# jamieapps101/Basic_Sparse_Matrix

Hardware: AMD Instinct MI355X
Metric: CSR x dense SpMM effective GB/s (B_alg / step time); nnz/s (higher is better)
Workload: dtype f64

## Files before the change

basic_sparse_matrix_amd/_lib.py:

```python

from __future__ import annotations

import ctypes
import os
import threading

import numpy as np

try:
    import torch
except Exception:
    torch = None

LIB_PATH = os.environ.get("BSM_LIB_PATH") or os.path.join(os.path.dirname(os.path.abspath(__file__)), "lib",
                                                          "libbsm_hip.so")

BSM_F64, BSM_F32, BSM_I32, BSM_U32, BSM_I64, BSM_U64 = range(6)
DTYPE_CODES = {
    np.dtype(np.float64): BSM_F64,
    np.dtype(np.float32): BSM_F32,
    np.dtype(np.int32): BSM_I32,
    np.dtype(np.uint32): BSM_U32,
    np.dtype(np.int64): BSM_I64,
    np.dtype(np.uint64): BSM_U64,
# ... 81 lines not shown
    ("bsm_dev_gen_row_ptr", _int, [_u64, _u64, _u64, _u32, _int, _u32, _u32, _vp, _vp, _u64, _vp]),
    ("bsm_dev_gen_entries", _int, [_int, _u64, _u64, _u64, _u32, _int, _vp, _vp, _vp, _vp]),
    ("bsm_dev_gen_dense", _int, [_int, _u64, _u64, _u64, _u64, _int, _vp, _vp]),
    ("bsm_dev_gen_insert_stream", _int, [_int, _u64, _u64, _u64, _u64, _u64, _u64, _vp, _vp, _vp, _vp]),
    ("bsm_dev_csr_from_inserts", _int, [_int, _u64, _u64, _u64, _vp, _vp, _vp, ctypes.POINTER(_vp), _vp]),
    ("bsm_dev_scan_workspace_bytes", _u64, [_u64]),
    ("bsm_dev_spmm", _int, [_int, _u64, _u64, _u64, _vp, _vp, _vp, _u64, _vp, _vp, _vp, _vp]),
    ("bsm_csr_panel_cols", _int, [_vp, _u64p]),
    ("bsm_dev_spmm_panel_cols", _u64, [_int, _u64, _u64]),
    ("bsm_dev_spmm_plan_bytes", _u64, [_u64, _u64, _u64]),
    ("bsm_dev_spmm_plan", _int, [_u64, _u64, _vp, _vp, _u64, _vp, ctypes.POINTER(_int), _vp]),
    ("bsm_dev_spmm_panelled", _int, [_int, _u64, _u64, _u64, _vp, _vp, _vp, _u64, _vp, _vp, _vp, _u64, _vp, _vp]),
    ("bsm_dev_tiled_wanted", _int, [_int, _u64, _u64, _u64, _u64, _u64]),
    ("bsm_dev_tiled_create", _int, [_u64, _u64, _u64, _vp, _vp, _vp, _u64, _int, ctypes.POINTER(_vp), _vp]),
    ("bsm_dev_spmm_tiled", _int, [_vp, _vp, _vp, _vp, _vp]),
    ("bsm_tiled_info", _int, [_vp, _u64p, _u64p, _u64p]),
    ("bsm_tiled_destroy", None, [_vp]),
    ("bsm_csr_tiled", _int, [_vp, ctypes.POINTER(_int)]),
    ("bsm_xfer_counters", _int, [_u64p]),
    ("bsm_xfer_counters_reset", None, []),
    ("bsm_dev_compact", _int, [_int, _u64, _u64, _vp, _vp, _vp, _vp, _vp, _vp, _u64, _vp]),
    ("bsm_multi_create", _int, [_int, ctypes.POINTER(_int), ctypes.POINTER(_vp)]),
    ("bsm_multi_unique_id", _int, [_vp]),
    ("bsm_multi_create_rank", _int, [_vp, _int, _int, _int, ctypes.POINTER(_vp)]),
    ("bsm_multi_create_external", _int, [_int, _int, _int, ctypes.POINTER(_vp)]),
    ("bsm_multi_is_external", _int, [_vp, ctypes.POINTER(_int)]),
    ("bsm_partition_rows", _int, [_vp, _u64, _u32, _vp]),
    ("bsm_multi_info", _int, [_vp, ctypes.POINTER(_int), ctypes.POINTER(_int), ctypes.POINTER(_int)]),
    ("bsm_multi_broadcast", _int, [_vp, _pp, _u64, _int]),
    ("bsm_multi_destroy", None, [_vp]),
    ("bsm_mcsr_upload", _int, [_vp, _int, _u64, _u64, _u64, _vp, _vp, _vp, _u32, ctypes.POINTER(_vp)]),
# ... 180 lines not shown
```

basic_sparse_matrix_amd/csrc/bsm_internal.hpp:

```cpp
#pragma once

#include <hip/hip_runtime.h>

#include <chrono>
#include <cstdint>
#include <cstdio>
#include <cstring>
#include <memory>
#include <mutex>
#include <string>

#include "../../include/bsm.h"

namespace bsm {

void set_error(const char* fmt, ...);
const char* last_error();
void stage_reset(hipStream_t s);
void stage_mark(const char* name, hipStream_t s);

#define BSM_HIP_TRY(expr)                                                                   \
    do {                                                                                    \
        hipError_t bsm_e_ = (expr);                                                         \
        if (bsm_e_ != hipSuccess) {                                                         \
// ... 132 lines not shown
        bytes = 0;
        cap = 0;
        return q;
    }
    template <typename T> T* as() const { return static_cast<T*>(p); }
};

}

struct bsm_tiled {
    int device = 0;
    int dtype = BSM_F64;
    uint64_t k = 32;
    uint32_t overread = 4;
    uint32_t stage = 4;
    uint64_t rows = 0, n_cols = 0, nnz = 0;
    uint32_t nw = 0, rpw = 0, nb = 0, rw = 0, pshift = 0;
    uint64_t chunks = 0;
    int64_t* offs = nullptr;
    void* meta = nullptr;
    uint32_t meta_bytes = 4;
    void* val = nullptr;
    unsigned* bar = nullptr;
};

struct bsm_csr {
    int dtype = BSM_F64;
    int device = 0;
    uint64_t rows = 0, cols = 0, nnz = 0;
    int64_t* row_ptr = nullptr;
// ... 68 lines not shown
                            const uint64_t* col, const void* vals, bsm_csr** out, hipStream_t s);
int sparse_addsub_dispatch(const bsm_csr* a, const bsm_csr* b, bool sub, bsm_csr** out, hipStream_t s);
int sparse_mul_dispatch(const bsm_csr* a, const bsm_csr* b, bsm_csr** out, hipStream_t s);
int csr_from_coo_device(int dtype, uint64_t rows, uint64_t cols, uint64_t n, const uint64_t* row,
                        const uint64_t* col, const void* vals, bsm_csr** out, hipStream_t s);
int gen_insert_stream(int dtype, uint64_t seed, uint64_t i0, uint64_t n, uint64_t rows, uint64_t cols,
                      uint64_t vmod, uint64_t* row, uint64_t* col, void* vals, hipStream_t s);
uint64_t spmm_panel_cols(int dtype, uint64_t n_cols, uint64_t k);
uint64_t spmm_plan_bytes(uint64_t rows, uint64_t n_cols, uint64_t panel_cols);
int spmm_plan(uint64_t rows, uint64_t n_cols, const int64_t* rp, const int32_t* col,
              uint64_t panel_cols, int32_t* seg, int* usable, hipStream_t s);
int spmm_panelled(int dtype, uint64_t rows, uint64_t n_cols, uint64_t nnz, const int64_t* rp,
                  const int32_t* col, const void* vals, uint64_t k, const void* x, void* y,
                  int32_t* row_nnz, uint64_t panel_cols, const int32_t* seg, hipStream_t s);
bool tiled_wanted(int dtype, uint64_t rows, uint64_t n_cols, uint64_t nnz, uint64_t k, uint64_t max_row_len);
int tiled_create(int dtype, uint64_t rows, uint64_t n_cols, uint64_t nnz, const int64_t* rp, const int32_t* col,
                 const void* vals, uint64_t k, int flags, bsm_tiled** out, hipStream_t s, uint64_t reserve = 0,
                 PlanTimes* pt = nullptr);
int tiled_spmm(const bsm_tiled* t, const void* x, void* y, int32_t* row_nnz, bool neg_init, hipStream_t s);
void tiled_destroy(bsm_tiled* t);
int compact_dispatch(int dtype, uint64_t rows, uint64_t k, const void* y, const int64_t* out_rp,
                     int32_t* out_col, void* out_vals, hipStream_t s);
constexpr uint64_t SMALL_OUT_ROWS = 8192;
constexpr uint64_t SMALL_OUT_CAP = 131072;
inline size_t small_col_bytes(uint64_t cap) { return (cap * sizeof(int32_t) + 15) / 16 * 16; }
int compact_small_dispatch(int dtype, uint64_t rows, uint64_t k, const int32_t* nz, const void* y, int64_t* out_rp,
                           int32_t* out_col, void* out_vals, void* host, uint64_t cap, hipStream_t s);
int pack_cols_to_rowmajor(int dtype, uint64_t n, uint64_t k, const void* colmajor, void* rowmajor,
                          hipStream_t s);
int unpack_rowmajor_to_cols(int dtype, uint64_t n, uint64_t k, const void* rowmajor,
// ... 29 lines not shown
```

basic_sparse_matrix_amd/csrc/capi.hip:

```cpp
#include <atomic>
#include <cstdarg>
#include <cstdlib>
#include <mutex>
#include <vector>

#include <algorithm>
#include <cstring>

#include "bsm_internal.hpp"

namespace bsm {

static thread_local std::string g_err;

void set_error(const char* fmt, ...) {
    char buf[1024];
    va_list ap;
    va_start(ap, fmt);
    vsnprintf(buf, sizeof(buf), fmt, ap);
    va_end(ap);
    g_err = buf;
}
const char* last_error() { return g_err.c_str(); }

// ... 1172 lines not shown
int bsm_dev_tiled_wanted(int dtype, uint64_t rows, uint64_t n_cols, uint64_t nnz, uint64_t k,
                         uint64_t max_row_len) {
    return tiled_wanted(dtype, rows, n_cols, nnz, k, max_row_len) ? 1 : 0;
}

int bsm_dev_tiled_create(uint64_t rows, uint64_t n_cols, uint64_t nnz, const int64_t* row_ptr,
                         const int32_t* col, const double* vals, uint64_t k, int flags, bsm_tiled** out,
                         void* stream) {
    return tiled_create(BSM_F64, rows, n_cols, nnz, row_ptr, col, vals, k, flags, out, static_cast<hipStream_t>(stream));
}

int bsm_dev_spmm_tiled(const bsm_tiled* t, const double* x, double* y, int32_t* row_nnz, void* stream) {
    return tiled_spmm(t, x, y, row_nnz, false, static_cast<hipStream_t>(stream));
}

int bsm_tiled_info(const bsm_tiled* t, uint64_t* bytes, uint64_t* slots, uint64_t* panel_cols) {
    BSM_REQUIRE(t, BSM_ERR_INVALID, "null argument");
    const uint64_t n = (t->chunks + t->overread) * 64;
    if (bytes) *bytes = n * (t->meta_bytes + (t->dtype == BSM_F32 ? 4 : 8)) + ((uint64_t)t->nw * t->nb + 1) * 8;
    if (slots) *slots = t->chunks * 64;
    if (panel_cols) *panel_cols = 1ull << t->pshift;
    return BSM_OK;
}

void bsm_tiled_destroy(bsm_tiled* t) { tiled_destroy(t); }

int bsm_csr_tiled(const bsm_csr* m, int* in_use) {
    BSM_REQUIRE(m && in_use, BSM_ERR_INVALID, "null argument");
    std::lock_guard<std::mutex> lock(m->plan_mu);
    *in_use = m->tiled ? 1 : 0;
    return BSM_OK;
}
// ... 12 lines not shown
```

basic_sparse_matrix_amd/csrc/kernels_tiled.hip:

```cpp
#include "bsm_internal.hpp"

#include <cstdlib>
#include <type_traits>
#include <utility>
#include <vector>


namespace bsm {
namespace {

constexpr int WAVE = 64;
constexpr int CHUNK = 64;
constexpr int PHASES = 6;
constexpr int OVERREAD = 4;
constexpr uint32_t DONE = 0xffffffffu;
constexpr uint32_t RW_MAX = 155;
constexpr uint32_t RW_MAX_F32 = 255;
constexpr uint32_t PSHIFT = 12;
constexpr uint32_t PACE_PCT = 3;

__device__ __forceinline__ uint64_t lanemask_lt(int lane) {
    return lane == 0 ? 0ull : (~0ull >> (64 - lane));
}
__device__ __forceinline__ uint32_t wave_min_u32(uint32_t v) {
#pragma unroll
    for (int off = 1; off < WAVE; off <<= 1) v = min(v, (uint32_t)__shfl_xor((int)v, off, WAVE));
    return v;
}

template <bool WRITE, int SLOTS, typename V, typename M = uint32_t>
__global__ __launch_bounds__(256) void tiled_layout(uint64_t rows, uint64_t n_cols, double pace, uint32_t rbits,
                                                    uint32_t pad, const int64_t* __restrict__ rp,
                                                    const int32_t* __restrict__ col,
                                                    const V* __restrict__ vals, uint32_t nw,
                                                    uint32_t rpw, uint32_t nb, uint32_t rw, uint32_t pshift,
                                                    int32_t* __restrict__ counts,
                                                    const int64_t* __restrict__ offs,
                                                    M* __restrict__ meta, V* __restrict__ val) {
    const int lane = threadIdx.x & (WAVE - 1);
    const uint64_t task = (uint64_t)blockIdx.x * (blockDim.x / WAVE) + threadIdx.x / WAVE;
    if (task >= (uint64_t)nw * nb) return;
    const uint64_t gw = task / nb, b = task % nb;
    const uint64_t w0 = gw * rpw;
    const uint64_t wend = min<uint64_t>(rows, w0 + rpw);
    const uint64_t r0 = w0 + b * rw;
// ... 1 lines not shown
    uint32_t h[SLOTS];
#pragma unroll
    for (int j = 0; j < SLOTS; ++j) {
        const uint32_t s = lane + WAVE * j;
        const bool live = s < rw && r0 + s < wend;
        cur[j] = live ? rp[r0 + s] : 0;
        end[j] = live ? rp[r0 + s + 1] : 0;
        h[j] = cur[j] < end[j] ? (uint32_t)col[cur[j]] >> pshift : DONE;
    }
    const bool any = r0 < wend;
    const int64_t t0 = any ? rp[r0] : 0, t1 = any ? rp[min<uint64_t>(r0 + rw, wend)] : 0;
    const double np = (double)(((n_cols - 1) >> pshift) + 1);
    const double inv_r = t1 > t0 ? (double)CHUNK * np / ((double)(t1 - t0) * pace) : 1e30;
    int64_t c = WRITE ? offs[task] : 0;
    int64_t n = 0;
    for (;;) {
        bool sel[SLOTS];
        int pos[SLOTS];
#pragma unroll
        for (int j = 0; j < SLOTS; ++j) {
            sel[j] = false;
            pos[j] = 0;
        }
        int taken = 0;
        const double pm = (double)n * inv_r;
        const uint32_t pmax = pm >= 4.0e9 ? DONE - 1 : (uint32_t)pm;
        bool done = false;
        while (taken < CHUNK) {
            uint32_t m = DONE;
#pragma unroll
            for (int j = 0; j < SLOTS; ++j) m = min(m, sel[j] ? DONE : h[j]);
            m = wave_min_u32(m);
            if (m == DONE) {
                done = taken == 0;
                break;
            }
            if (m > pmax) break;
            int before = 0;
#pragma unroll
            for (int j = 0; j < SLOTS; ++j) {
                const bool cand = !sel[j] && h[j] == m;
                const uint64_t bal = __ballot(cand);
                const int rank = before + __popcll(bal & lanemask_lt(lane));
                if (cand && taken + rank < CHUNK) {
                    sel[j] = true;
                    pos[j] = taken + rank;
                }
                before += __popcll(bal);
            }
            taken = min(taken + before, CHUNK);
        }
        if (done) break;
#pragma unroll
        for (int j = 0; j < SLOTS; ++j) {
            if (sel[j]) {
                const int64_t e = cur[j];
                if (WRITE) {
                    meta[c * CHUNK + pos[j]] = ((M)(uint32_t)col[e] << rbits) | (M)(lane + WAVE * j);
                    val[c * CHUNK + pos[j]] = vals[e];
                }
                cur[j] = e + 1;
                h[j] = cur[j] < end[j] ? (uint32_t)col[cur[j]] >> pshift : DONE;
            }
        }
        if (WRITE && lane >= taken) {
            meta[c * CHUNK + lane] = (M)rw;
            val[c * CHUNK + lane] = (V)0;
        }
        ++c;
        ++n;
    }
    const int64_t padded = (n + pad - 1) / pad * pad;
    if (WRITE) {
        for (int64_t p = n; p < padded; ++p, ++c) {
            meta[c * CHUNK + lane] = (M)rw;
            val[c * CHUNK + lane] = (V)0;
        }
    } else if (lane == 0) {
        counts[task] = (int32_t)padded;
    }
}

template <typename T> struct Vec2;
template <> struct Vec2<double> { using type = double2; };
struct F2 {
    uint64_t u;
};
template <> struct Vec2<float> { using type = F2; };
__device__ __forceinline__ double lo_of(const double2& v) { return v.x; }
__device__ __forceinline__ double hi_of(const double2& v) { return v.y; }
// ... 140 lines not shown
}

template <bool PROBE, typename T = double, typename M = uint32_t>
__global__ __launch_bounds__(256) __attribute__((amdgpu_waves_per_eu(1, 1))) void spmm_tiled_k32(
    uint64_t rows, uint32_t rpw, uint32_t nb, uint32_t rw, const int64_t* __restrict__ offs,
    const M* __restrict__ meta, const T* __restrict__ val, const vec2_t<T>* __restrict__ X,
    vec2_t<T>* __restrict__ Y, int32_t* __restrict__ row_nnz, unsigned* bar, uint32_t xmask, uint32_t spins) {
    spmm_tiled_k32_body<PROBE, T, M>(rows, rpw, nb, rw, offs, meta, val, X, Y, row_nnz, bar, xmask, spins);
}
template <typename M = uint32_t>
__global__ __launch_bounds__(256) __attribute__((amdgpu_waves_per_eu(1, 1))) void spmm_tiled_k32_f32(
    uint64_t rows, uint32_t rpw, uint32_t nb, uint32_t rw, const int64_t* __restrict__ offs,
    const M* __restrict__ meta, const float* __restrict__ val, const F2* __restrict__ X, F2* __restrict__ Y,
    int32_t* __restrict__ row_nnz, unsigned* bar, uint32_t xmask, uint32_t spins) {
    spmm_tiled_k32_body<false, float, M>(rows, rpw, nb, rw, offs, meta, val, X, Y, row_nnz, bar, xmask, spins);
}

constexpr int K1_STAGE_DEFAULT = 4;
constexpr uint32_t K1_RBITS = 11;
constexpr uint32_t K1_RW_MAX = (1u << K1_RBITS) - 1;
constexpr uint32_t K1_PSHIFT = 18;
constexpr uint32_t K1_WAVES_PER_CU = 4;

template <int ST, typename T>
struct Stage1 {
    uint32_t m[ST];
    T v[ST];
    T x[ST];
};
template <int ST, typename T>
// ... 96 lines not shown

bool tiled_wanted(int dtype, uint64_t rows, uint64_t n_cols, uint64_t nnz, uint64_t k, uint64_t max_row_len) {
    const bool shape = (dtype == BSM_F64 || dtype == BSM_F32) && rows > 0 && nnz > 0 &&
                       ((k == 32 && n_cols <= 0x7fffffffull) || (k == 1 && n_cols < (1u << (32 - K1_RBITS))));
    if (const char* e = getenv("BSM_SPMM_TILED")) {
        if (atoi(e) == 0) return false;
        if (atoi(e) == 2) return shape;
    }
    if (!shape) return false;
    const uint64_t x_bytes = n_cols * k * (dtype == BSM_F32 ? 4 : 8);
    if (x_bytes <= (k == 32 ? (1ull << 30) : (4ull << 20))) return false;
    const uint64_t mean = (nnz + rows - 1) / rows;
    return max_row_len <= 2 * mean + 256;
}

int tiled_create(int dtype, uint64_t rows, uint64_t n_cols, uint64_t nnz, const int64_t* rp, const int32_t* col,
                 const void* vals, uint64_t k, int flags, bsm_tiled** out, hipStream_t s, uint64_t reserve,
                 PlanTimes* pt) {
    BSM_REQUIRE(out && rp && (nnz == 0 || (col && vals)), BSM_ERR_INVALID, "tiled: null argument");
    BSM_REQUIRE(k == 32 || k == 1, BSM_ERR_UNSUPPORTED, "tiled: k must be 32 or 1");
    BSM_REQUIRE(dtype == BSM_F64 || dtype == BSM_F32, BSM_ERR_UNSUPPORTED, "tiled: f64 or f32 only");
    const bool f32 = dtype == BSM_F32;
    const size_t es = f32 ? 4 : 8;
    const bool wide = k == 32 && n_cols >= (1ull << 24);
    const size_t mb = wide ? 8 : 4;
    const uint32_t rbits = k == 1 ? K1_RBITS : 8;
    BSM_REQUIRE(k == 32 ? n_cols <= 0x7fffffffull : n_cols < (1ull << (32 - rbits)), BSM_ERR_UNSUPPORTED,
                "tiled: columns must be < 2^%u", k == 32 ? 31u : 32 - rbits);
    *out = nullptr;
    int dev = 0;
// ... 2 lines not shown
    BSM_HIP_TRY(hipDeviceGetAttribute(&cus, hipDeviceAttributeMultiprocessorCount, dev));
    if (s && cus > 0) {
        std::vector<uint32_t> mk((size_t)(cus + 31) / 32, 0u);
        if (hipExtStreamGetCUMask(s, (uint32_t)mk.size(), mk.data()) == hipSuccess) {
            int n = 0;
            for (int i = 0; i < cus; ++i) n += (mk[i / 32] >> (i % 32)) & 1u;
            if (n > 0 && n < cus) cus = n;
        } else {
            (void)hipGetLastError();
        }
    }
    const uint32_t wpc = k == 1 ? K1_WAVES_PER_CU : 4u;
    const uint32_t nw_env = env_u32("BSM_TILED_WAVES", wpc * (uint32_t)cus);
    const uint32_t nw = nw_env;
    const uint32_t k1_stage = env_u32("BSM_TILED_K1_STAGE", K1_STAGE_DEFAULT) == 8 ? 8u : 4u;
    const uint32_t rw_cap =
        k == 1 ? K1_RW_MAX : (f32 ? RW_MAX_F32 : RW_MAX);
    uint32_t rw_max = env_u32("BSM_TILED_RW", rw_cap);
    rw_max = rw_max < 8u ? 8u : (rw_max > rw_cap ? rw_cap : rw_max);
    const uint32_t pshift = env_u32("BSM_TILED_PSHIFT", k == 1 ? K1_PSHIFT : PSHIFT);
    const double pace = 1.0 + env_u32("BSM_TILED_PACE_PCT", PACE_PCT) / 100.0;
    const uint32_t pad = k == 1 ? 1u : PHASES;
    const uint32_t overread = k == 1 ? 2 * k1_stage : OVERREAD;
    BSM_REQUIRE(nw >= wpc && nw % wpc == 0 && pshift < 32, BSM_ERR_INVALID, "tiled: bad geometry");
    const uint64_t rpw64 = (rows + nw - 1) / nw;
    BSM_REQUIRE(rpw64 < (1ull << 31), BSM_ERR_UNSUPPORTED, "tiled: too many rows per wave");
    const uint32_t rpw = rpw64 ? (uint32_t)rpw64 : 1u;
    const uint32_t nb = (rpw + rw_max - 1) / rw_max;
    const uint32_t rw = (rpw + nb - 1) / nb;
    const uint64_t tasks = (uint64_t)nw * nb;

    DBuf counts, offs, ws;
    BSM_TRY(counts.alloc(tasks * sizeof(int32_t)));
    BSM_TRY(offs.alloc((tasks + 1) * sizeof(int64_t)));
    const uint64_t grid = (tasks + 3) / 4;
    auto layout = [&](auto write_tag, int32_t* cnt, const int64_t* of, void* me, void* va) -> int {
        constexpr bool W = decltype(write_tag)::value;
        auto go = [&]<typename V, typename MT>(V*, MT*) {
            if (k == 1)
                tiled_layout<W, (K1_RW_MAX + 1) / WAVE, V, MT><<<dim3((unsigned)grid), 256, 0, s>>>(
                    rows, n_cols, pace, rbits, pad, rp, col, static_cast<const V*>(vals), nw, rpw, nb, rw, pshift,
                    cnt, of, static_cast<MT*>(me), static_cast<V*>(va));
            else if (rw_cap > 192)
                tiled_layout<W, 4, V, MT><<<dim3((unsigned)grid), 256, 0, s>>>(
                    rows, n_cols, pace, rbits, pad, rp, col, static_cast<const V*>(vals), nw, rpw, nb, rw, pshift,
                    cnt, of, static_cast<MT*>(me), static_cast<V*>(va));
            else
                tiled_layout<W, 3, V, MT><<<dim3((unsigned)grid), 256, 0, s>>>(
                    rows, n_cols, pace, rbits, pad, rp, col, static_cast<const V*>(vals), nw, rpw, nb, rw, pshift,
                    cnt, of, static_cast<MT*>(me), static_cast<V*>(va));
        };
        if (f32 && wide) go((float*)nullptr, (uint64_t*)nullptr);
        else if (f32) go((float*)nullptr, (uint32_t*)nullptr);
        else if (wide) go((double*)nullptr, (uint64_t*)nullptr);
        else go((double*)nullptr, (uint32_t*)nullptr);
        BSM_HIP_TRY(hipGetLastError());
        return BSM_OK;
    };
// ... 36 lines not shown
    auto* t = new bsm_tiled;
    t->device = dev;
    t->dtype = dtype;
    t->k = k;
    t->rows = rows;
    t->n_cols = n_cols;
    t->nnz = nnz;
    t->nw = nw;
    t->rpw = rpw;
    t->nb = nb;
    t->rw = rw;
    t->pshift = pshift;
    t->chunks = (uint64_t)total;
    t->overread = overread;
    t->stage = k1_stage;
    t->offs = static_cast<int64_t*>(offs.release());
    t->meta_bytes = (uint32_t)mb;
    t->meta = meta.release();
    t->val = val.release();
    t->bar = static_cast<unsigned*>(bar.release());
    *out = t;
    return BSM_OK;
}

int tiled_spmm(const bsm_tiled* t, const void* x, void* y, int32_t* row_nnz, bool neg_init, hipStream_t s) {
    BSM_REQUIRE(t && (t->rows == 0 || (x && y)), BSM_ERR_INVALID, "tiled: null argument");
    BSM_REQUIRE(!neg_init || t->k == 1, BSM_ERR_INVALID, "tiled: -0 init only for k = 1");
    if (t->rows == 0) return BSM_OK;
    unsigned* bar = nullptr;
    if (t->bar && t->nb > 1 && env_u32("BSM_TILED_SYNC", 1)) {
        BSM_HIP_TRY(hipMemsetAsync(t->bar, 0, 8 * BAR_STRIDE * sizeof(unsigned), s));
        bar = t->bar;
    }
    static const uint32_t k1mask = env_u32("BSM_TILED_K1_PROBE", 0xffffffffu);
    if (t->k == 1 && t->dtype == BSM_F32) {
        const size_t lds = (size_t)4 * (t->rw + 1) * sizeof(float);
        auto kern = t->stage == 8 ? spmm_tiled_k1<8, float> : spmm_tiled_k1<4, float>;
        kern<<<dim3(t->nw / 4), 256, lds, s>>>(t->rows, t->rpw, t->nb, t->rw, t->offs,
                                              static_cast<const uint32_t*>(t->meta),
                                              static_cast<const float*>(t->val), static_cast<const float*>(x),
                                              static_cast<float*>(y), row_nnz, bar, neg_init, k1mask);
    } else if (t->k == 1) {
        const size_t lds = (size_t)4 * (t->rw + 1) * sizeof(double);
        auto kern = t->stage == 8 ? spmm_tiled_k1<8> : spmm_tiled_k1<4>;
        kern<<<dim3(t->nw / 4), 256, lds, s>>>(t->rows, t->rpw, t->nb, t->rw, t->offs,
// ... 7 lines not shown
            spmm_tiled_k32_f32<uint64_t><<<dim3(t->nw / 4), 256, lds, s>>>(
                t->rows, t->rpw, t->nb, t->rw, t->offs, static_cast<const uint64_t*>(t->meta),
                static_cast<const float*>(t->val), static_cast<const F2*>(x), static_cast<F2*>(y), row_nnz,
                bar, 0xffffffffu, spins);
        else
            spmm_tiled_k32_f32<uint32_t><<<dim3(t->nw / 4), 256, lds, s>>>(
                t->rows, t->rpw, t->nb, t->rw, t->offs, static_cast<const uint32_t*>(t->meta),
                static_cast<const float*>(t->val), static_cast<const F2*>(x), static_cast<F2*>(y), row_nnz,
                bar, 0xffffffffu, spins);
    } else {
        const size_t lds = (size_t)4 * (t->rw + 1) * 256;
        static const uint32_t xmask = env_u32("BSM_TILED_PROBE_MASK", 0xffffffffu);
        auto kern = xmask != 0xffffffffu ? spmm_tiled_k32<true>
                                         : spmm_tiled_k32<false>;
        static const uint32_t spins = env_u32("BSM_TILED_SPINS", 4000);
        if (t->meta_bytes == 8)
            spmm_tiled_k32<false, double, uint64_t><<<dim3(t->nw / 4), 256, lds, s>>>(
                t->rows, t->rpw, t->nb, t->rw, t->offs, static_cast<const uint64_t*>(t->meta),
                static_cast<const double*>(t->val), static_cast<const double2*>(x), static_cast<double2*>(y), row_nnz,
                bar, 0xffffffffu, spins);
        else
            kern<<<dim3(t->nw / 4), 256, lds, s>>>(t->rows, t->rpw, t->nb, t->rw, t->offs,
                                                  static_cast<const uint32_t*>(t->meta),
                                                  static_cast<const double*>(t->val), static_cast<const double2*>(x),
                                                  static_cast<double2*>(y), row_nnz, bar, xmask, spins);
    }
    BSM_HIP_TRY(hipGetLastError());
    return BSM_OK;
}

void tiled_destroy(bsm_tiled* t) {
// ... 10 lines not shown
```

basic_sparse_matrix_amd/csrc/multi.hip:

```cpp
#include <rccl/rccl.h>

#include <algorithm>
#include <mutex>
#include <string>
#include <thread>
#include <vector>

#include "bsm_internal.hpp"

#define BSM_NCCL_TRY(expr)                                                                              \
    do {                                                                                                \
        ncclResult_t bsm_r_ = (expr);                                                                   \
        if (bsm_r_ != ncclSuccess) {                                                                    \
            ::bsm::set_error("%s failed: %s (%s:%d)", #expr, ncclGetErrorString(bsm_r_), __FILE__,     \
                             __LINE__);                                                                 \
            return BSM_ERR_COMM;                                                                        \
        }                                                                                               \
    } while (0)

struct bsm_multi {
    int world = 1, first_rank = 0, n_local = 0;
    bool external = false;
    std::vector<int> devices;
    std::vector<ncclComm_t> comms;
// ... 593 lines not shown
}

int bsm_mcsr_plan_info(const bsm_mcsr* m, int* tiled_pieces, int* local_pieces, uint64_t* copy_bytes,
                       uint64_t* panel_cols) {
    BSM_REQUIRE(m, BSM_ERR_INVALID, "null handle");
    std::lock_guard<std::recursive_mutex> hold(m->mu);
    int nt = 0, np = 0;
    uint64_t bytes = 0, pc = 0;
    for (const auto& L : m->loc)
        for (const bsm_csr* a : L.pieces) {
            std::lock_guard<std::mutex> lk(a->plan_mu);
            ++np;
            if (m->prepared && m->schedule != 2 && a->tiled && a->tiled->k == m->k) {
                ++nt;
                uint64_t b = 0, w = 0;
                (void)bsm_tiled_info(a->tiled, &b, nullptr, &w);
                bytes += b;
                pc = w;
            } else if (a->plan_usable && !pc) {
                pc = a->plan_cols;
            }
        }
    if (tiled_pieces) *tiled_pieces = nt;
    if (local_pieces) *local_pieces = np;
    if (copy_bytes) *copy_bytes = bytes;
    if (panel_cols) *panel_cols = pc;
    return BSM_OK;
}

int bsm_mcsr_step(bsm_mcsr* m, const void* const* x_dev) {
    BSM_REQUIRE(m, BSM_ERR_INVALID, "bsm_mcsr_step: null handle");
// ... 284 lines not shown
```

basic_sparse_matrix_amd/device.py:

```python

from __future__ import annotations

import ctypes
from dataclasses import dataclass

import numpy as np
import torch

from . import _lib

TORCH_DT = {
    np.dtype(np.float64): torch.float64,
    np.dtype(np.float32): torch.float32,
    np.dtype(np.int32): torch.int32,
    np.dtype(np.uint32): torch.uint32,
    np.dtype(np.int64): torch.int64,
    np.dtype(np.uint64): torch.uint64,
}


def _stream(stream=None) -> int:
    s = stream if stream is not None else torch.cuda.current_stream()
    return s.cuda_stream

# ... 88 lines not shown
            return
        _lib.check(lib.bsm_dev_spmm(_lib.DTYPE_CODES[self.dtype], self.rows, self.n_cols, self.nnz, _p(self.row_ptr),
                                    _p(self.col), _p(self.vals), k, _p(x), _p(y),
                                    _p(row_nnz) if row_nnz is not None else 0, _stream(stream)))


class TiledPlan:

    def __init__(self, handle: int, k: int = 32):
        self.handle = handle
        self.k = k

    def info(self) -> dict:
        lib = _lib.load()
        b, sl, pc = ctypes.c_uint64(), ctypes.c_uint64(), ctypes.c_uint64()
        _lib.check(lib.bsm_tiled_info(self.handle, ctypes.byref(b), ctypes.byref(sl), ctypes.byref(pc)))
        return {"bytes": b.value, "slots": sl.value, "panel_cols": pc.value}

    def __del__(self):
        if getattr(self, "handle", None) and _lib._lib is not None:
            _lib._lib.bsm_tiled_destroy(self.handle)
            self.handle = None


def gen_dense(seed, row0, n, k, value_kind=_lib.VAL_UNIFORM, dtype=np.float64, device="cuda") -> torch.Tensor:
    lib = _lib.require_device()
    dt = np.dtype(dtype)
    x = torch.empty((n, k), dtype=TORCH_DT[dt], device=device)
    _lib.check(lib.bsm_dev_gen_dense(_lib.DTYPE_CODES[dt], seed, row0, n, k, value_kind, _p(x), _stream()))
    return x


# ... 84 lines not shown
```

include/bsm.h:

```cpp
#ifndef BSM_H
#define BSM_H

#include <stdint.h>

#ifdef __cplusplus
extern "C" {
#endif

#define BSM_API_VERSION 1

typedef enum bsm_dtype {
    BSM_F64 = 0,
    BSM_F32 = 1,
    BSM_I32 = 2,
    BSM_U32 = 3,
    BSM_I64 = 4,
    BSM_U64 = 5
} bsm_dtype;

typedef enum bsm_status {
    BSM_OK = 0,
    BSM_ERR_INVALID = 1,
    BSM_ERR_DIMENSIONS = 2,
    BSM_ERR_NON_SQUARE = 3,
// ... 97 lines not shown
int bsm_dev_spmm_plan(uint64_t rows, uint64_t n_cols, const int64_t* row_ptr, const int32_t* col,
                      uint64_t panel_cols, int32_t* seg, int* usable, void* stream);
int bsm_dev_spmm_panelled(int dtype, uint64_t rows, uint64_t n_cols, uint64_t nnz,
                          const int64_t* row_ptr, const int32_t* col, const void* vals, uint64_t k,
                          const void* x, void* y, int32_t* row_nnz, uint64_t panel_cols,
                          const int32_t* seg, void* stream);
typedef struct bsm_tiled bsm_tiled;
#define BSM_TILED_ANY_PADDING 1
int bsm_dev_tiled_wanted(int dtype, uint64_t rows, uint64_t n_cols, uint64_t nnz, uint64_t k,
                         uint64_t max_row_len);
int bsm_dev_tiled_create(uint64_t rows, uint64_t n_cols, uint64_t nnz, const int64_t* row_ptr,
                         const int32_t* col, const double* vals, uint64_t k, int flags,
                         bsm_tiled** out, void* stream);
int bsm_dev_spmm_tiled(const bsm_tiled* t, const double* x, double* y, int32_t* row_nnz,
                       void* stream);
int bsm_tiled_info(const bsm_tiled* t, uint64_t* bytes, uint64_t* slots, uint64_t* panel_cols);
int bsm_csr_tiled(const bsm_csr* m, int* in_use);
int bsm_xfer_counters(uint64_t out[8]);
void bsm_xfer_counters_reset(void);
void bsm_tiled_destroy(bsm_tiled* t);
int bsm_dev_compact(int dtype, uint64_t rows, uint64_t k, const void* y,
                    const int32_t* row_nnz, int64_t* out_row_ptr, int32_t* out_col,
                    void* out_vals, void* workspace, uint64_t workspace_bytes, void* stream);

typedef struct bsm_multi bsm_multi;
typedef struct bsm_mcsr bsm_mcsr;
#define BSM_UNIQUE_ID_BYTES 128
int bsm_multi_create(int n_gpus, const int* devices, bsm_multi** out);
int bsm_multi_unique_id(void* id);
int bsm_multi_create_rank(const void* id, int world, int rank, int device, bsm_multi** out);
int bsm_multi_create_external(int world, int rank, int device, bsm_multi** out);
// ... 35 lines not shown
```

Before: 686.2.

## Add two-pass half-width tiled SpMM kernel for f64 k=32 with larger row batches

Adds a tiled SpMM path for f64 with k=32 that splits the 32 output columns into two 16-column halves, each handled in its own pass. Halving the per-row scratch lets each batch cover up to twice as many rows (310 instead of 155), which is meant to give more reuse of each gathered X row within a batch. The layout kernel interleaves entries into even/odd lane classes, and the compute kernel broadcasts indices and values with DPP. A heuristic based on expected column collisions picks the mode automatically, and an env var can override it. The cost is reading meta and values twice and doubling the barrier syncs.

```diff
diff --git a/basic_sparse_matrix_amd/_lib.py b/basic_sparse_matrix_amd/_lib.py
--- a/basic_sparse_matrix_amd/_lib.py
+++ b/basic_sparse_matrix_amd/_lib.py
@@ -119,7 +119,9 @@
     ("bsm_dev_tiled_wanted", _int, [_int, _u64, _u64, _u64, _u64, _u64]),
     ("bsm_dev_tiled_create", _int, [_u64, _u64, _u64, _vp, _vp, _vp, _u64, _int, ctypes.POINTER(_vp), _vp]),
     ("bsm_dev_spmm_tiled", _int, [_vp, _vp, _vp, _vp, _vp]),
-    ("bsm_tiled_info", _int, [_vp, _u64p, _u64p, _u64p]),
+    ("bsm_dev_tiled_half_wanted", _int, [_int, _u64, _u64, _u64, _u64, ctypes.c_uint32]),
+    ("bsm_tiled_info", _int, [_vp, _u64p, _u64p, _u64p, ctypes.POINTER(ctypes.c_uint32),
+                              ctypes.POINTER(ctypes.c_uint32)]),
     ("bsm_tiled_destroy", None, [_vp]),
     ("bsm_csr_tiled", _int, [_vp, ctypes.POINTER(_int)]),
     ("bsm_xfer_counters", _int, [_u64p]),
diff --git a/basic_sparse_matrix_amd/csrc/bsm_internal.hpp b/basic_sparse_matrix_amd/csrc/bsm_internal.hpp
--- a/basic_sparse_matrix_amd/csrc/bsm_internal.hpp
+++ b/basic_sparse_matrix_amd/csrc/bsm_internal.hpp
@@ -170,6 +170,7 @@
     uint64_t k = 32;
     uint32_t overread = 4;
     uint32_t stage = 4;
+    uint32_t passes = 1;
     uint64_t rows = 0, n_cols = 0, nnz = 0;
     uint32_t nw = 0, rpw = 0, nb = 0, rw = 0, pshift = 0;
     uint64_t chunks = 0;
@@ -268,6 +269,7 @@
                   const int32_t* col, const void* vals, uint64_t k, const void* x, void* y,
                   int32_t* row_nnz, uint64_t panel_cols, const int32_t* seg, hipStream_t s);
 bool tiled_wanted(int dtype, uint64_t rows, uint64_t n_cols, uint64_t nnz, uint64_t k, uint64_t max_row_len);
+bool tiled_half_wanted(int dtype, uint64_t rows, uint64_t n_cols, uint64_t nnz, uint64_t k, uint32_t cus);
 int tiled_create(int dtype, uint64_t rows, uint64_t n_cols, uint64_t nnz, const int64_t* rp, const int32_t* col,
                  const void* vals, uint64_t k, int flags, bsm_tiled** out, hipStream_t s, uint64_t reserve = 0,
                  PlanTimes* pt = nullptr);
diff --git a/basic_sparse_matrix_amd/csrc/capi.hip b/basic_sparse_matrix_amd/csrc/capi.hip
--- a/basic_sparse_matrix_amd/csrc/capi.hip
+++ b/basic_sparse_matrix_amd/csrc/capi.hip
@@ -1210,8 +1210,15 @@
     return tiled_spmm(t, x, y, row_nnz, false, static_cast<hipStream_t>(stream));
 }
 
-int bsm_tiled_info(const bsm_tiled* t, uint64_t* bytes, uint64_t* slots, uint64_t* panel_cols) {
+int bsm_dev_tiled_half_wanted(int dtype, uint64_t rows, uint64_t n_cols, uint64_t nnz, uint64_t k, uint32_t cus) {
+    return tiled_half_wanted(dtype, rows, n_cols, nnz, k, cus) ? 1 : 0;
+}
+
+int bsm_tiled_info(const bsm_tiled* t, uint64_t* bytes, uint64_t* slots, uint64_t* panel_cols, uint32_t* passes,
+                   uint32_t* batch_rows) {
     BSM_REQUIRE(t, BSM_ERR_INVALID, "null argument");
+    if (passes) *passes = t->passes;
+    if (batch_rows) *batch_rows = t->rw;
     const uint64_t n = (t->chunks + t->overread) * 64;
     if (bytes) *bytes = n * (t->meta_bytes + (t->dtype == BSM_F32 ? 4 : 8)) + ((uint64_t)t->nw * t->nb + 1) * 8;
     if (slots) *slots = t->chunks * 64;
diff --git a/basic_sparse_matrix_amd/csrc/kernels_tiled.hip b/basic_sparse_matrix_amd/csrc/kernels_tiled.hip
--- a/basic_sparse_matrix_amd/csrc/kernels_tiled.hip
+++ b/basic_sparse_matrix_amd/csrc/kernels_tiled.hip
@@ -1,5 +1,6 @@
 #include "bsm_internal.hpp"
 
+#include <cmath>
 #include <cstdlib>
 #include <type_traits>
 #include <utility>
@@ -16,9 +17,16 @@
 constexpr uint32_t DONE = 0xffffffffu;
 constexpr uint32_t RW_MAX = 155;
 constexpr uint32_t RW_MAX_F32 = 255;
+constexpr uint32_t RW_MAX_HALF = 310;
+constexpr int H_GATHER_AHEAD = 1;
+constexpr int H_IDX_AHEAD = 2;
+constexpr int H_XRING = H_GATHER_AHEAD + 1, H_IRING = 2 * H_XRING;
+constexpr int PHASES_HALF = H_IRING;
+constexpr int OVERREAD_HALF = H_IDX_AHEAD;
 constexpr uint32_t PSHIFT = 12;
 constexpr uint32_t PACE_PCT = 3;
 
+__host__ __device__ constexpr uint32_t half_scratch_row(uint32_t rw) { return (rw + 1) & ~1u; }
 __device__ __forceinline__ uint64_t lanemask_lt(int lane) {
     return lane == 0 ? 0ull : (~0ull >> (64 - lane));
 }
@@ -28,7 +36,7 @@
     return v;
 }
 
-template <bool WRITE, int SLOTS, typename V, typename M = uint32_t>
+template <bool WRITE, int SLOTS, typename V, typename M = uint32_t, bool HALF = false>
 __global__ __launch_bounds__(256) void tiled_layout(uint64_t rows, uint64_t n_cols, double pace, uint32_t rbits,
                                                     uint32_t pad, const int64_t* __restrict__ rp,
                                                     const int32_t* __restrict__ col,
@@ -60,6 +68,7 @@
     const double inv_r = t1 > t0 ? (double)CHUNK * np / ((double)(t1 - t0) * pace) : 1e30;
     int64_t c = WRITE ? offs[task] : 0;
     int64_t n = 0;
+    const M dummy = HALF ? (M)(half_scratch_row(rw) >> 1) : (M)rw;
     for (;;) {
         bool sel[SLOTS];
         int pos[SLOTS];
@@ -68,33 +77,43 @@
             sel[j] = false;
             pos[j] = 0;
         }
-        int taken = 0;
+        constexpr int NCLS = HALF ? 2 : 1;
+        constexpr int CAP = CHUNK / NCLS;
+        int taken[NCLS];
         const double pm = (double)n * inv_r;
         const uint32_t pmax = pm >= 4.0e9 ? DONE - 1 : (uint32_t)pm;
-        bool done = false;
-        while (taken < CHUNK) {
-            uint32_t m = DONE;
-#pragma unroll
-            for (int j = 0; j < SLOTS; ++j) m = min(m, sel[j] ? DONE : h[j]);
-            m = wave_min_u32(m);
-            if (m == DONE) {
-                done = taken == 0;
-                break;
+        bool done = true;
+#pragma unroll
+        for (int cls = 0; cls < NCLS; ++cls) {
+            const bool mine = !HALF || (lane & 1) == cls;
+            int tk = 0;
+            bool fin = false;
+            while (tk < CAP) {
+                uint32_t m = DONE;
+#pragma unroll
+                for (int j = 0; j < SLOTS; ++j) m = min(m, (sel[j] || !mine) ? DONE : h[j]);
+                m = wave_min_u32(m);
+                if (m == DONE) {
+                    fin = tk == 0;
+                    break;
+                }
+                if (m > pmax) break;
+                int before = 0;
+#pragma unroll
+                for (int j = 0; j < SLOTS; ++j) {
+                    const bool cand = mine && !sel[j] && h[j] == m;
+                    const uint64_t bal = __ballot(cand);
+                    const int rank = before + __popcll(bal & lanemask_lt(lane));
+                    if (cand && tk + rank < CAP) {
+                        sel[j] = true;
+                        pos[j] = HALF ? 2 * (tk + rank) + cls : tk + rank;
+                    }
+                    before += __popcll(bal);
+                }
+                tk = min(tk + before, CAP);
             }
-            if (m > pmax) break;
-            int before = 0;
-#pragma unroll
-            for (int j = 0; j < SLOTS; ++j) {
-                const bool cand = !sel[j] && h[j] == m;
-                const uint64_t bal = __ballot(cand);
-                const int rank = before + __popcll(bal & lanemask_lt(lane));
-                if (cand && taken + rank < CHUNK) {
-                    sel[j] = true;
-                    pos[j] = taken + rank;
-                }
-                before += __popcll(bal);
-            }
-            taken = min(taken + before, CHUNK);
+            done = done && fin;
+            taken[cls] = tk;
         }
         if (done) break;
 #pragma unroll
@@ -102,15 +121,16 @@
             if (sel[j]) {
                 const int64_t e = cur[j];
                 if (WRITE) {
-                    meta[c * CHUNK + pos[j]] = ((M)(uint32_t)col[e] << rbits) | (M)(lane + WAVE * j);
+                    const uint32_t slot = lane + WAVE * j;
+                    meta[c * CHUNK + pos[j]] = ((M)(uint32_t)col[e] << rbits) | (M)(HALF ? slot >> 1 : slot);
                     val[c * CHUNK + pos[j]] = vals[e];
                 }
                 cur[j] = e + 1;
                 h[j] = cur[j] < end[j] ? (uint32_t)col[cur[j]] >> pshift : DONE;
             }
         }
-        if (WRITE && lane >= taken) {
-            meta[c * CHUNK + lane] = (M)rw;
+        if (WRITE && (HALF ? (lane >> 1) >= taken[lane & (NCLS - 1)] : lane >= taken[0])) {
+            meta[c * CHUNK + lane] = dummy;
             val[c * CHUNK + lane] = (V)0;
         }
         ++c;
@@ -119,7 +139,7 @@
     const int64_t padded = (n + pad - 1) / pad * pad;
     if (WRITE) {
         for (int64_t p = n; p < padded; ++p, ++c) {
-            meta[c * CHUNK + lane] = (M)rw;
+            meta[c * CHUNK + lane] = dummy;
             val[c * CHUNK + lane] = (V)0;
         }
     } else if (lane == 0) {
@@ -290,6 +310,109 @@
     const M* __restrict__ meta, const float* __restrict__ val, const F2* __restrict__ X, F2* __restrict__ Y,
     int32_t* __restrict__ row_nnz, unsigned* bar, uint32_t xmask, uint32_t spins) {
     spmm_tiled_k32_body<false, float, M>(rows, rpw, nb, rw, offs, meta, val, X, Y, row_nnz, bar, xmask, spins);
+}
+
+template <int U>
+__device__ __forceinline__ uint32_t bm8(uint32_t mi) {
+    const int a = __builtin_amdgcn_mov_dpp((int)mi, 0x150 + 2 * U, 0xf, 0x3, false);
+    return (uint32_t)__builtin_amdgcn_update_dpp(a, (int)mi, 0x150 + 2 * U + 1, 0xf, 0xc, false);
+}
+template <int U>
+__device__ __forceinline__ double bv8(double vi) {
+    const int lo = __builtin_amdgcn_mov_dpp(__double2loint(vi), 0x150 + 2 * U, 0xf, 0x3, false);
+    const int hi = __builtin_amdgcn_mov_dpp(__double2hiint(vi), 0x150 + 2 * U, 0xf, 0x3, false);
+    return __hiloint2double(__builtin_amdgcn_update_dpp(hi, __double2hiint(vi), 0x150 + 2 * U + 1, 0xf, 0xc, false),
+                            __builtin_amdgcn_update_dpp(lo, __double2loint(vi), 0x150 + 2 * U + 1, 0xf, 0xc, false));
+}
+template <bool PROBE, int... U>
+__device__ __forceinline__ void gather_half(double2 (&x)[8], uint32_t (&mb)[8], const Idx<double>& c,
+                                            const char* __restrict__ Xh, uint32_t j16, uint32_t xmask,
+                                            std::integer_sequence<int, U...>) {
+    ((mb[U] = bm8<U>(c.mi)), ...);
+    if (PROBE) ((x[U] = *reinterpret_cast<const double2*>(Xh + ((((mb[U] >> 8) & xmask) << 8) | j16))), ...);
+    else ((x[U] = *reinterpret_cast<const double2*>(Xh + ((mb[U] & 0xffffff00u) | j16))), ...);
+}
+__device__ __forceinline__ double2* yaddr_half(uint32_t mb, double2* ys) {
+    return reinterpret_cast<double2*>(reinterpret_cast<char*>(ys) + ((mb & 255u) << 8));
+}
+template <int U>
+__device__ __forceinline__ void madd_half(double2& y, const double2& x, const Idx<double>& c) {
+    const double v = bv8<U>(c.vi);
+    y = make_double2(__dadd_rn(y.x, __dmul_rn(v, x.x)), __dadd_rn(y.y, __dmul_rn(v, x.y)));
+}
+template <int... U>
+__device__ __forceinline__ void sum_chunk_half(const double2 (&x)[8], const uint32_t (&mb)[8], const Idx<double>& c,
+                                               double2* ys, std::integer_sequence<int, U...>) {
+    double2 y[8];
+    ((y[U] = *yaddr_half(mb[U], ys)), ...);
+    (madd_half<U>(y[U], x[U], c), ...);
+    ((*yaddr_half(mb[U], ys) = y[U]), ...);
+}
+
+template <bool PROBE>
+__global__ __launch_bounds__(256) __attribute__((amdgpu_waves_per_eu(1, 1))) void spmm_tiled_k32_half(
+    uint64_t rows, uint32_t rpw, uint32_t nb, uint32_t rw, const int64_t* __restrict__ offs,
+    const uint32_t* __restrict__ meta, const double* __restrict__ val, const double2* __restrict__ X,
+    double2* __restrict__ Y, int32_t* __restrict__ row_nnz, unsigned* bar, uint32_t xmask, uint32_t spins) {
+    extern __shared__ __align__(16) unsigned char yhalf_raw[];
+    double2* const yhalf = reinterpret_cast<double2*>(yhalf_raw);
+    const int lane = threadIdx.x & (WAVE - 1);
+    const int wave = threadIdx.x / WAVE;
+    const int g = lane >> 3, j = lane & 7;
+    double2* yw = yhalf + (size_t)wave * (half_scratch_row(rw) + 2) * 8;
+    double2* ys = yw + (g & 1) * 8 + j;
+    const uint64_t gw = (uint64_t)blockIdx.x * (blockDim.x / WAVE) + wave;
+    const uint64_t w0 = gw * rpw;
+    const uint64_t wend = min<uint64_t>(rows, w0 + rpw);
+    const uint32_t waves = gridDim.x * (blockDim.x / WAVE);
+    constexpr auto SEQ = std::make_integer_sequence<int, 8>{};
+    bool sync = bar != nullptr;
+    for (uint32_t st = 0; st < 2 * nb; ++st) {
+        const uint32_t b = st >> 1, h = st & 1;
+        const uint64_t r0 = w0 + (uint64_t)b * rw;
+        if (r0 >= wend) {
+            if (sync) batch_arrive(bar, 2 * nb - st, lane);
+            break;
+        }
+        if (sync && st > 0) sync = batch_wait(bar, waves * st, lane, spins);
+        const int nr = (int)min<uint64_t>(rw, wend - r0);
+        for (int r = g; r < nr; r += 8) yw[r * 8 + j] = make_double2(0.0, 0.0);
+        const char* Xh = reinterpret_cast<const char*>(X) + 128 * h;
+        const uint32_t j16 = 16 * j;
+        const int64_t c0 = offs[gw * nb + b], c1 = offs[gw * nb + b + 1];
+        if (c1 > c0) {
+            Idx<double> MI[H_IRING];
+            double2 XS[H_XRING][8];
+            uint32_t MB[H_XRING][8];
+#pragma unroll
+            for (int k = 0; k < H_IDX_AHEAD; ++k) load_idx(MI[k], meta, val, c0 + k, lane);
+#pragma unroll
+            for (int k = 0; k < H_GATHER_AHEAD; ++k) gather_half<PROBE>(XS[k], MB[k], MI[k], Xh, j16, xmask, SEQ);
+            for (int64_t i = c0; i < c1; i += PHASES_HALF) {
+#pragma unroll
+                for (int k = 0; k < PHASES_HALF; ++k) {
+                    load_idx(MI[(k + H_IDX_AHEAD) % H_IRING], meta, val, i + k + H_IDX_AHEAD, lane);
+                    gather_half<PROBE>(XS[(k + H_GATHER_AHEAD) % H_XRING], MB[(k + H_GATHER_AHEAD) % H_XRING],
+                                       MI[(k + H_GATHER_AHEAD) % H_IRING], Xh, j16, xmask, SEQ);
+                    __builtin_amdgcn_sched_barrier(0);
+                    sum_chunk_half(XS[k % H_XRING], MB[k % H_XRING], MI[k], ys, SEQ);
+                    __builtin_amdgcn_sched_barrier(0);
+                }
+            }
+        }
+        for (int rb = 0; rb < nr; rb += 8) {
+            const int r = rb + g;
+            const bool live = r < nr;
+            const double2 y = live ? yw[r * 8 + j] : make_double2(0.0, 0.0);
+            if (live) Y[(r0 + r) * 16 + 8 * h + j] = y;
+            const uint64_t m0 = __ballot(y.x != 0.0), m1 = __ballot(y.y != 0.0);
+            if (live && j == 0 && row_nnz) {
+                const int n = __popcll((m0 >> (8 * g)) & 0xffull) + __popcll((m1 >> (8 * g)) & 0xffull);
+                row_nnz[r0 + r] = h ? row_nnz[r0 + r] + n : n;
+            }
+        }
+        if (sync) batch_arrive(bar, 1, lane);
+    }
 }
 
 constexpr int K1_STAGE_DEFAULT = 4;
@@ -416,6 +539,13 @@
     return max_row_len <= 2 * mean + 256;
 }
 
+bool tiled_half_wanted(int dtype, uint64_t rows, uint64_t n_cols, uint64_t nnz, uint64_t k, uint32_t cus) {
+    if (dtype != BSM_F64 || k != 32 || n_cols >= (1ull << 24) || rows == 0 || n_cols == 0 || nnz == 0) return false;
+    const double lam = (double)cus / 8.0 * 4.0 * (double)RW_MAX * (double)nnz / ((double)rows * (double)n_cols);
+    auto f = [](double l) { return l < 1e-9 ? 1.0 : -std::expm1(-l) / l; };
+    return f(lam) - f(2.0 * lam) > 12.0 / 256.0;
+}
+
 int tiled_create(int dtype, uint64_t rows, uint64_t n_cols, uint64_t nnz, const int64_t* rp, const int32_t* col,
                  const void* vals, uint64_t k, int flags, bsm_tiled** out, hipStream_t s, uint64_t reserve,
                  PlanTimes* pt) {
@@ -448,14 +578,17 @@
     const uint32_t nw_env = env_u32("BSM_TILED_WAVES", wpc * (uint32_t)cus);
     const uint32_t nw = nw_env;
     const uint32_t k1_stage = env_u32("BSM_TILED_K1_STAGE", K1_STAGE_DEFAULT) == 8 ? 8u : 4u;
+    const bool half_ok = k == 32 && !f32 && !wide;
+    const bool half = half_ok && env_u32("BSM_TILED_HALF", tiled_half_wanted(dtype, rows, n_cols, nnz, k,
+                                                                              (uint32_t)cus)) != 0;
     const uint32_t rw_cap =
-        k == 1 ? K1_RW_MAX : (f32 ? RW_MAX_F32 : RW_MAX);
+        k == 1 ? K1_RW_MAX : (f32 ? RW_MAX_F32 : (half ? RW_MAX_HALF : RW_MAX));
     uint32_t rw_max = env_u32("BSM_TILED_RW", rw_cap);
     rw_max = rw_max < 8u ? 8u : (rw_max > rw_cap ? rw_cap : rw_max);
     const uint32_t pshift = env_u32("BSM_TILED_PSHIFT", k == 1 ? K1_PSHIFT : PSHIFT);
     const double pace = 1.0 + env_u32("BSM_TILED_PACE_PCT", PACE_PCT) / 100.0;
-    const uint32_t pad = k == 1 ? 1u : PHASES;
-    const uint32_t overread = k == 1 ? 2 * k1_stage : OVERREAD;
+    const uint32_t pad = k == 1 ? 1u : (half ? PHASES_HALF : PHASES);
+    const uint32_t overread = k == 1 ? 2 * k1_stage : (half ? OVERREAD_HALF : OVERREAD);
     BSM_REQUIRE(nw >= wpc && nw % wpc == 0 && pshift < 32, BSM_ERR_INVALID, "tiled: bad geometry");
     const uint64_t rpw64 = (rows + nw - 1) / nw;
     BSM_REQUIRE(rpw64 < (1ull << 31), BSM_ERR_UNSUPPORTED, "tiled: too many rows per wave");
@@ -475,7 +608,16 @@
                 tiled_layout<W, (K1_RW_MAX + 1) / WAVE, V, MT><<<dim3((unsigned)grid), 256, 0, s>>>(
                     rows, n_cols, pace, rbits, pad, rp, col, static_cast<const V*>(vals), nw, rpw, nb, rw, pshift,
                     cnt, of, static_cast<MT*>(me), static_cast<V*>(va));
-            else if (rw_cap > 192)
+            else if constexpr (std::is_same_v<V, double> && std::is_same_v<MT, uint32_t>) {
+                if (half)
+                    tiled_layout<W, 5, V, MT, true><<<dim3((unsigned)grid), 256, 0, s>>>(
+                        rows, n_cols, pace, rbits, pad, rp, col, static_cast<const V*>(vals), nw, rpw, nb, rw,
+                        pshift, cnt, of, static_cast<MT*>(me), static_cast<V*>(va));
+                else
+                    tiled_layout<W, 3, V, MT><<<dim3((unsigned)grid), 256, 0, s>>>(
+                        rows, n_cols, pace, rbits, pad, rp, col, static_cast<const V*>(vals), nw, rpw, nb, rw,
+                        pshift, cnt, of, static_cast<MT*>(me), static_cast<V*>(va));
+            } else if (rw_cap > 192)
                 tiled_layout<W, 4, V, MT><<<dim3((unsigned)grid), 256, 0, s>>>(
                     rows, n_cols, pace, rbits, pad, rp, col, static_cast<const V*>(vals), nw, rpw, nb, rw, pshift,
                     cnt, of, static_cast<MT*>(me), static_cast<V*>(va));
@@ -542,6 +684,7 @@
     t->chunks = (uint64_t)total;
     t->overread = overread;
     t->stage = k1_stage;
+    t->passes = half ? 2u : 1u;
     t->offs = static_cast<int64_t*>(offs.release());
     t->meta_bytes = (uint32_t)mb;
     t->meta = meta.release();
@@ -556,7 +699,7 @@
     BSM_REQUIRE(!neg_init || t->k == 1, BSM_ERR_INVALID, "tiled: -0 init only for k = 1");
     if (t->rows == 0) return BSM_OK;
     unsigned* bar = nullptr;
-    if (t->bar && t->nb > 1 && env_u32("BSM_TILED_SYNC", 1)) {
+    if (t->bar && t->nb * t->passes > 1 && env_u32("BSM_TILED_SYNC", 1)) {
         BSM_HIP_TRY(hipMemsetAsync(t->bar, 0, 8 * BAR_STRIDE * sizeof(unsigned), s));
         bar = t->bar;
     }
@@ -594,7 +737,14 @@
         auto kern = xmask != 0xffffffffu ? spmm_tiled_k32<true>
                                          : spmm_tiled_k32<false>;
         static const uint32_t spins = env_u32("BSM_TILED_SPINS", 4000);
-        if (t->meta_bytes == 8)
+        if (t->passes == 2) {
+            const size_t lds_half = (size_t)4 * (half_scratch_row(t->rw) + 2) * 128;
+            auto kern_half = xmask != 0xffffffffu ? spmm_tiled_k32_half<true> : spmm_tiled_k32_half<false>;
+            kern_half<<<dim3(t->nw / 4), 256, lds_half, s>>>(
+                t->rows, t->rpw, t->nb, t->rw, t->offs, static_cast<const uint32_t*>(t->meta),
+                static_cast<const double*>(t->val), static_cast<const double2*>(x), static_cast<double2*>(y), row_nnz,
+                bar, xmask, spins);
+        } else if (t->meta_bytes == 8)
             spmm_tiled_k32<false, double, uint64_t><<<dim3(t->nw / 4), 256, lds, s>>>(
                 t->rows, t->rpw, t->nb, t->rw, t->offs, static_cast<const uint64_t*>(t->meta),
                 static_cast<const double*>(t->val), static_cast<const double2*>(x), static_cast<double2*>(y), row_nnz,
diff --git a/basic_sparse_matrix_amd/csrc/multi.hip b/basic_sparse_matrix_amd/csrc/multi.hip
--- a/basic_sparse_matrix_amd/csrc/multi.hip
+++ b/basic_sparse_matrix_amd/csrc/multi.hip
@@ -631,7 +631,7 @@
             if (m->prepared && m->schedule != 2 && a->tiled && a->tiled->k == m->k) {
                 ++nt;
                 uint64_t b = 0, w = 0;
-                (void)bsm_tiled_info(a->tiled, &b, nullptr, &w);
+                (void)bsm_tiled_info(a->tiled, &b, nullptr, &w, nullptr, nullptr);
                 bytes += b;
                 pc = w;
             } else if (a->plan_usable && !pc) {
diff --git a/basic_sparse_matrix_amd/device.py b/basic_sparse_matrix_amd/device.py
--- a/basic_sparse_matrix_amd/device.py
+++ b/basic_sparse_matrix_amd/device.py
@@ -126,8 +126,11 @@
     def info(self) -> dict:
         lib = _lib.load()
         b, sl, pc = ctypes.c_uint64(), ctypes.c_uint64(), ctypes.c_uint64()
-        _lib.check(lib.bsm_tiled_info(self.handle, ctypes.byref(b), ctypes.byref(sl), ctypes.byref(pc)))
-        return {"bytes": b.value, "slots": sl.value, "panel_cols": pc.value}
+        ps, br = ctypes.c_uint32(), ctypes.c_uint32()
+        _lib.check(lib.bsm_tiled_info(self.handle, ctypes.byref(b), ctypes.byref(sl), ctypes.byref(pc),
+                                      ctypes.byref(ps), ctypes.byref(br)))
+        return {"bytes": b.value, "slots": sl.value, "panel_cols": pc.value, "passes": ps.value,
+                "batch_rows": br.value}
 
     def __del__(self):
         if getattr(self, "handle", None) and _lib._lib is not None:
diff --git a/include/bsm.h b/include/bsm.h
--- a/include/bsm.h
+++ b/include/bsm.h
@@ -135,7 +135,10 @@
                          bsm_tiled** out, void* stream);
 int bsm_dev_spmm_tiled(const bsm_tiled* t, const double* x, double* y, int32_t* row_nnz,
                        void* stream);
-int bsm_tiled_info(const bsm_tiled* t, uint64_t* bytes, uint64_t* slots, uint64_t* panel_cols);
+int bsm_dev_tiled_half_wanted(int dtype, uint64_t rows, uint64_t n_cols, uint64_t nnz, uint64_t k,
+                              uint32_t cus);
+int bsm_tiled_info(const bsm_tiled* t, uint64_t* bytes, uint64_t* slots, uint64_t* panel_cols,
+                   uint32_t* passes, uint32_t* batch_rows);
 int bsm_csr_tiled(const bsm_csr* m, int* in_use);
 int bsm_xfer_counters(uint64_t out[8]);
 void bsm_xfer_counters_reset(void);
```

Measured after the change: 731.8, median of 6. 1.07x the previous value.
